# monkey0head/RePlay_cql

Hardware: AMD Instinct MI355X
Metric: CQL train-steps/sec (higher is better)
Workload: dtype bf16; 1 GPU; BASELINE.json configs[2]: synthetic 1000000 users x 100000 items, CQL d=128, L=50, B=4096/GPU, bf16 MFMA + fp32 accumulate; users=1000000, items=100000, d=128, window=50, batch_per_gpu=4096, global_batch=4096, parallelism=dp1 (users sharded by rank, RCCL gradient all-reduce), k=10, dp_variant=single

## Files before the change

### include/cqlrec.h

```cpp
#ifndef CQLREC_H
#define CQLREC_H
#include <stdint.h>
#ifdef __cplusplus
extern "C" {
#endif

#define CQLREC_OK 0
#define CQLREC_ERR_INVALID (-1)
#define CQLREC_ERR_HIP (-2)
#define CQLREC_ABI_VERSION 2
#define CQLREC_SEG_ALIGN 64

typedef void* cqlrec_stream;

int cqlrec_abi_version(void);
const char* cqlrec_last_error(void);

typedef struct cqlrec_layout {
  int64_t n_items;
  int32_t d;
  int32_t reserved;
  int64_t off_E_in, off_E_out, off_b_out, off_W1, off_b1, off_W2, off_b2;
  int64_t total;
} cqlrec_layout;
int cqlrec_layout_make(int64_t n_items, int32_t d, cqlrec_layout* out );

int cqlrec_sample_transitions(const int64_t* offsets, const int32_t* items, const float* rewards, int64_t n_users,
                              uint64_t seed, uint64_t step, uint64_t slot0, int32_t batch, int32_t* users,
                              int32_t* tpos, int32_t* act, float* rew, float* done, cqlrec_stream stream);

int cqlrec_gather_pool_fwd(const uint16_t* E_in_b, const int64_t* offsets, const int32_t* items,
                           const int32_t* users, const int32_t* ends, int32_t end_delta, int64_t n_states,
                           int32_t L, int32_t d, float* h0, uint16_t* h0_b, int32_t* lens, cqlrec_stream stream);
int cqlrec_gather_pool_bwd(const float* dh0, const int64_t* offsets, const int32_t* items, const int32_t* users,
                           const int32_t* ends, int32_t end_delta, int64_t n_states, int32_t L, int32_t d,
                           float* g_E_in, cqlrec_stream stream);
int64_t cqlrec_gather_pool_bwd_ws_bytes(int64_t n_states, int32_t L, int32_t d);
int cqlrec_gather_pool_bwd_prepare(const int64_t* offsets, const int32_t* items, const int32_t* users,
                                   const int32_t* ends, int32_t end_delta, int64_t n_states, int32_t L, int32_t d,
                                   int64_t n_items, void* ws, int64_t ws_bytes, cqlrec_stream stream);
int cqlrec_gather_pool_bwd_apply(const float* dh0, int64_t n_states, int32_t L, int32_t d, int64_t n_items, void* ws,
                                 int64_t ws_bytes, float* g_E_in, cqlrec_stream stream);
int cqlrec_gather_pool_bwd_sorted(const float* dh0, const int64_t* offsets, const int32_t* items,
                                  const int32_t* users, const int32_t* ends, int32_t end_delta, int64_t n_states,
                                  int32_t L, int32_t d, int64_t n_items, void* ws, int64_t ws_bytes,
                                  float* g_E_in, cqlrec_stream stream);

int cqlrec_linear_bf16(const uint16_t* X_b, const uint16_t* W_b, const float* bias, int64_t rows, int32_t d,
                       int32_t relu, float* Y, uint16_t* Y_b, cqlrec_stream stream);
int cqlrec_encoder_fwd(const uint16_t* X_b, const uint16_t* W1_b, const float* b1, const uint16_t* W2_b, const float* b2,
                       int64_t rows, int32_t d, uint16_t* Z_b, uint16_t* H_b, cqlrec_stream stream);
int64_t cqlrec_encoder_bwd_ws_bytes(int64_t rows, int32_t d);
int cqlrec_encoder_bwd(const float* dH, const uint16_t* z_b, const uint16_t* h0_b, const uint16_t* W1_b,
                       const uint16_t* W2_b, int64_t rows, int32_t d, void* ws, int64_t ws_bytes, float* g_W1,
                       float* g_b1, float* g_W2, float* g_b2, float* dh0, cqlrec_stream stream);

#define CQLREC_QHEAD_LSE 1
#define CQLREC_QHEAD_ARGMAX 2
int64_t cqlrec_qhead_ws_bytes(int64_t rows, int64_t n_items, int32_t d);
int cqlrec_qhead_fwd(const uint16_t* H_b, int64_t rows, const uint16_t* E_out_b, const float* b_out,
                     int64_t n_items, int32_t d, int32_t mode, void* ws, int64_t ws_bytes, float* out_val,
                     int32_t* out_idx, float* out_nlse2, cqlrec_stream stream);

int cqlrec_gather_dot(const uint16_t* H_b, const uint16_t* E_b, const float* b, const int32_t* idx, int64_t rows,
                      int32_t d, float* out, cqlrec_stream stream);

int cqlrec_td_loss(const float* q_a, const float* lse, const float* q_targ, const float* rew, const float* done,
                   int32_t batch, float gamma, float alpha, float inv_batch, float* coef, float* y,
                   float* loss_out, cqlrec_stream stream);
int64_t cqlrec_qhead_bwd_ws_bytes(int64_t batch, int64_t n_items, int32_t d);
int cqlrec_qhead_bwd(const uint16_t* H_b, const float* nlse2, const float* coef, const int32_t* act,
                     int64_t batch, const uint16_t* E_out_b, const float* b_out, int64_t n_items, int32_t d,
                     float scale, void* ws, int64_t ws_bytes, float* dH, float* g_E_out, float* g_b_out,
                     cqlrec_stream stream);

int cqlrec_qhead_bwd_items(const uint16_t* H_b, const float* nlse2, const float* coef, const int32_t* act,
                           int64_t batch, const uint16_t* E_out_b, const float* b_out, int64_t n_items, int32_t d,
                           float scale, void* ws, int64_t ws_bytes, float* g_E_out, float* g_b_out,
                           cqlrec_stream stream);
int cqlrec_qhead_bwd_states(const uint16_t* H_b, const float* nlse2, const float* coef, const int32_t* act,
                            int64_t batch, const uint16_t* E_out_b, const float* b_out, int64_t n_items, int32_t d,
                            float scale, void* ws, int64_t ws_bytes, float* dH, cqlrec_stream stream);

int64_t cqlrec_qhead_fused_ws_bytes(int64_t rows, int64_t n_items, int32_t d);
int cqlrec_qhead_fwd_lse_dh(const uint16_t* H_b, int64_t rows, const uint16_t* E_out_b, const float* b_out,
                            int64_t n_items, int32_t d, void* ws, int64_t ws_bytes, float* out_lse,
                            float* out_nlse2 , cqlrec_stream stream);
int cqlrec_qhead_dh_finish(const void* ws, int64_t rows, int64_t n_items, int32_t d, const float* lse,
                           const float* coef, const int32_t* act, const uint16_t* E_out_b, float scale, float* dH,
                           cqlrec_stream stream);

int cqlrec_adam_ema(float* theta, float* grads, float* m, float* v, float* target, uint16_t* theta_b,
                    uint16_t* target_b, int64_t n, float step_size, float sqrt_bc2, float beta1, float beta2,
                    float eps, float tau, int32_t zero_grads, cqlrec_stream stream);
int cqlrec_cast_bf16(const float* src, uint16_t* dst_b, int64_t n, cqlrec_stream stream);

int64_t cqlrec_topk_ws_bytes(int64_t n_users, int64_t n_cand, int32_t d, int32_t k);
int cqlrec_score_topk(const uint16_t* H_b, int64_t n_users, const uint16_t* E_b, const float* b, int64_t n_cand,
                      int32_t d, const int32_t* item_ids, const int64_t* seen_off, const int32_t* seen_items,
                      const int32_t* seen_rows, int32_t k, void* ws, int64_t ws_bytes, int32_t* out_idx,
                      float* out_val, int32_t* out_cnt, cqlrec_stream stream);
#define CQLREC_TOPK_ALL 0
#define CQLREC_TOPK_SEEN 1
#define CQLREC_TOPK_SCORE 2
// ... 339 lines not shown
```

### replay_cql_amd/_native.py

```python
from __future__ import annotations

import ctypes as C
import os
from pathlib import Path
from typing import Optional

os.environ.setdefault("GPU_MAX_HW_QUEUES", "8")

_LIB_PATH = Path(os.environ["CQLREC_LIB"]).resolve() if os.environ.get("CQLREC_LIB") else \
    Path(__file__).resolve().parent / "libcqlrec.so"
_lib: Optional[C.CDLL] = None

ABI_VERSION = 2
TOPK_ALL, TOPK_SEEN, TOPK_SCORE, TOPK_SEEN_BESIDE = 0, 1, 2, 3
SIM_DOT, SIM_COSINE, SIM_EUCLID = 0, 1, 2
ITEM_KNN_MAX_K = 512
PAIRS_MAX_K = 512
QHEAD_LSE = 1
QHEAD_ARGMAX = 2
EVAL_EXTRAS = ("RocAuc", "Unexpectedness", "Surprisal", "NCISPrecision")
NCIS_NONE, NCIS_SIGMOID, NCIS_SOFTMAX = 0, 1, 2

vp, i32, i64, u64, f32, f64 = C.c_void_p, C.c_int32, C.c_int64, C.c_uint64, C.c_float, C.c_double


class Layout(C.Structure):
    _fields_ = [
        ("n_items", i64), ("d", i32), ("reserved", i32),
        ("off_E_in", i64), ("off_E_out", i64), ("off_b_out", i64), ("off_W1", i64), ("off_b1", i64),
        ("off_W2", i64), ("off_b2", i64), ("total", i64),
    ]

    SEGMENTS = ("E_in", "E_out", "b_out", "W1", "b1", "W2", "b2")

    def offset(self, name: str) -> int:
        return int(getattr(self, "off_" + name))

    def shape(self, name: str):
        n, d = int(self.n_items), int(self.d)
        return {"E_in": (n + 1, d), "E_out": (n, d), "b_out": (n,), "W1": (d, d), "b1": (d,), "W2": (d, d),
                "b2": (d,)}[name]


class TrainCtx(C.Structure):
    _fields_ = [
        ("layout", Layout),
        ("offsets", vp), ("items", vp), ("rewards", vp), ("n_users", i64),
        ("theta", vp), ("grads", vp), ("adam_m", vp), ("adam_v", vp), ("target", vp), ("theta_b", vp),
        ("target_b", vp),
        ("batch", i32), ("window", i32), ("world", i32), ("rank", i32),
        ("gamma", f64), ("alpha", f64), ("lr", f64), ("beta1", f64), ("beta2", f64), ("eps", f64), ("tau", f64),
        ("seed", u64),
        ("ws", vp), ("ws_bytes", i64),
    ]


class TrainViews(C.Structure):
    _fields_ = [(n, vp) for n in (
        "users", "tpos", "act", "a_star", "rew", "done", "q_a", "lse", "q_targ", "y", "coef", "dH", "dh0", "h0_s",
        "hb_s", "hb_sn", "hb_tn")]


class FeaturesPop(C.Structure):
    _fields_ = [("code", vp), ("pair_code", vp), ("keys", vp), ("pop", vp), ("entity_off", vp), ("n_code", i64), ("n_entity", i64),
                ("n_cat", i64), ("m", i64), ("entity_is_item", i32), ("reserved", i32)]


FEATURES_STATS, FEATURES_MAX_COLS, FEATURES_MAX_POP = 6, 64, 8
FEAT_MEAN_GATHER, FEAT_MEAN_ABNORMALITY, FEAT_MEAN_ABNORMALITY_CR = 0, 1, 2
(FEAT_COL_USER, FEAT_COL_ITEM, FEAT_COL_NA_USER, FEAT_COL_NA_ITEM, FEAT_COL_DIFF_USER, FEAT_COL_DIFF_ITEM, FEAT_COL_POP,
 FEAT_COL_POP_NA) = range(8)

NEIGHBOUR_FIT, NEIGHBOUR_PREDICT = 0, 1
NEIGHBOUR_MAX_K = 1024
NEIGHBOUR_WEIGHTINGS = {None: 0, "tf_idf": 1, "bm25": 2}

ALS_PIECE, ALS_GRAM_BLOCK, ALS_MAX_RANK, ALS_MAX_K = 1024, 4096, 128, 512
ALS_EXPLICIT, ALS_IMPLICIT = 0, 1

SIGNATURES = {
    "cqlrec_abi_version": (i32, []),
    "cqlrec_last_error": (C.c_char_p, []),
    "cqlrec_layout_make": (i32, [i64, i32, C.POINTER(Layout)]),
    "cqlrec_sample_transitions": (i32, [vp, vp, vp, i64, u64, u64, u64, i32, vp, vp, vp, vp, vp, vp]),
    "cqlrec_gather_pool_fwd": (i32, [vp, vp, vp, vp, vp, i32, i64, i32, i32, vp, vp, vp, vp]),
    "cqlrec_gather_pool_bwd": (i32, [vp, vp, vp, vp, vp, i32, i64, i32, i32, vp, vp]),
    "cqlrec_gather_pool_bwd_ws_bytes": (i64, [i64, i32, i32]),
    "cqlrec_gather_pool_bwd_prepare": (i32, [vp, vp, vp, vp, i32, i64, i32, i32, i64, vp, i64, vp]),
    "cqlrec_gather_pool_bwd_apply": (i32, [vp, i64, i32, i32, i64, vp, i64, vp, vp]),
    "cqlrec_gather_pool_bwd_sorted": (i32, [vp, vp, vp, vp, vp, i32, i64, i32, i32, i64, vp, i64, vp, vp]),
    "cqlrec_linear_bf16": (i32, [vp, vp, vp, i64, i32, i32, vp, vp, vp]),
    "cqlrec_encoder_fwd": (i32, [vp, vp, vp, vp, vp, i64, i32, vp, vp, vp]),
    "cqlrec_encoder_bwd_ws_bytes": (i64, [i64, i32]),
    "cqlrec_encoder_bwd": (i32, [vp, vp, vp, vp, vp, i64, i32, vp, i64, vp, vp, vp, vp, vp, vp]),
    "cqlrec_qhead_ws_bytes": (i64, [i64, i64, i32]),
    "cqlrec_qhead_fwd": (i32, [vp, i64, vp, vp, i64, i32, i32, vp, i64, vp, vp, vp, vp]),
    "cqlrec_gather_dot": (i32, [vp, vp, vp, vp, i64, i32, vp, vp]),
    "cqlrec_td_loss": (i32, [vp, vp, vp, vp, vp, i32, f32, f32, f32, vp, vp, vp, vp]),
    "cqlrec_qhead_bwd_ws_bytes": (i64, [i64, i64, i32]),
    "cqlrec_qhead_bwd": (i32, [vp, vp, vp, vp, i64, vp, vp, i64, i32, f32, vp, i64, vp, vp, vp, vp]),
    "cqlrec_qhead_bwd_items": (i32, [vp, vp, vp, vp, i64, vp, vp, i64, i32, f32, vp, i64, vp, vp, vp]),
    "cqlrec_qhead_bwd_states": (i32, [vp, vp, vp, vp, i64, vp, vp, i64, i32, f32, vp, i64, vp, vp]),
    "cqlrec_adam_ema": (i32, [vp, vp, vp, vp, vp, vp, vp, i64, f32, f32, f32, f32, f32, f32, i32, vp]),
    "cqlrec_cast_bf16": (i32, [vp, vp, i64, vp]),
    "cqlrec_topk_ws_bytes": (i64, [i64, i64, i32, i32]),
    "cqlrec_score_topk": (i32, [vp, i64, vp, vp, i64, i32, vp, vp, vp, vp, i32, vp, i64, vp, vp, vp, vp]),
    "cqlrec_topk_seen_form": (i32, [vp, i64, i64, i32, i32, C.POINTER(C.c_int32), vp]),
    "cqlrec_score_topk_phase": (i32, [vp, i64, vp, vp, i64, i32, vp, vp, vp, vp, i32, vp, i64, vp, vp, vp, i32, vp]),
    "cqlrec_item_norms": (i32, [vp, i64, i32, vp, vp]),
    "cqlrec_item_knn_ws_bytes": (i64, [i64, i64, i32, i32]),
    "cqlrec_item_knn": (i32, [vp, vp, i64, i32, vp, i64, vp, i64, i32, i32, vp, i64, vp, vp, vp, vp]),
    "cqlrec_pairs_topk_ws_bytes": (i64, [i64, i64, i32, i32]),
    "cqlrec_pairs_topk": (i32, [vp, vp, vp, i64, i32, vp, vp, vp, i64, vp, vp, i32, vp, i64, vp, vp, vp, vp, vp]),
    "cqlrec_train_ws_bytes": (i64, [i32, i64, i32, i32]),
    "cqlrec_train_step_fwd_bwd": (i32, [C.POINTER(TrainCtx), u64, vp, vp]),
    "cqlrec_train_step_update": (i32, [C.POINTER(TrainCtx), u64, vp]),
    "cqlrec_train_step_forward": (i32, [C.POINTER(TrainCtx), u64, vp, vp]),
    "cqlrec_train_step_forward_after": (i32, [C.POINTER(TrainCtx), u64, vp, vp, vp]),
    "cqlrec_train_step_forward_early_items": (i32, [C.POINTER(TrainCtx), u64, vp, vp, vp, vp]),
    "cqlrec_train_step_backward_items": (i32, [C.POINTER(TrainCtx), u64, vp]),
    "cqlrec_train_step_backward_rest": (i32, [C.POINTER(TrainCtx), u64, vp]),
    "cqlrec_train_step_update_range": (i32, [C.POINTER(TrainCtx), u64, i64, i64, vp]),
    "cqlrec_set_concurrency": (i32, [i32]),
    "cqlrec_runtime_init": (i32, []),
    "cqlrec_runtime_probe_count": (i32, []),
    "cqlrec_aux_stream": (vp, [i32]),
    "cqlrec_qhead_fused_ws_bytes": (i64, [i64, i64, i32]),
    "cqlrec_qhead_fwd_lse_dh": (i32, [vp, i64, vp, vp, i64, i32, vp, i64, vp, vp, vp]),
    "cqlrec_qhead_dh_finish": (i32, [vp, i64, i64, i32, vp, vp, vp, vp, C.c_float, vp, vp]),
    "cqlrec_train_steps": (i32, [C.POINTER(TrainCtx), u64, i32, vp, vp]),
    "cqlrec_train_views_get": (i32, [C.POINTER(TrainCtx), u64, C.POINTER(TrainViews)]),
    "cqlrec_build_csr_ws_bytes": (i64, [i64]),
    "cqlrec_build_csr": (i32, [vp, vp, vp, vp, i64, i64, vp, i64, vp, vp, vp, vp]),
    "cqlrec_eval_topk_ws_bytes": (i64, [i64, i32]),
    "cqlrec_eval_topk": (i32, [vp, i64, i32, vp, vp, vp, C.POINTER(i32), i32, vp, i64, vp, vp, vp]),
    "cqlrec_recs_frame_to_block_ws_bytes": (i64, [i64, i64]),
    "cqlrec_recs_frame_to_block": (i32, [vp, vp, vp, vp, i64, i64, i32, i32, vp, i64, vp, vp, vp, vp, vp]),
    "cqlrec_recs_join_prev": (i32, [vp, vp, i64, vp, vp, i64, vp, vp]),
# ... 143 lines not shown
```

### replay_cql_amd/csrc/common.h

```cpp
#pragma once
#include <hip/hip_runtime.h>
#include <stdint.h>
#include <stdio.h>
#include <stdarg.h>

#include "../../include/cqlrec.h"

typedef __attribute__((ext_vector_type(8))) __bf16 bf16x8;
typedef __attribute__((ext_vector_type(4))) __bf16 bf16x4;
typedef __attribute__((ext_vector_type(16))) float f32x16;
typedef __attribute__((ext_vector_type(4))) float f32x4;
typedef __attribute__((address_space(3))) bf16x4 lds_bf16x4;

#define CQL_WAVE 64
#define CQL_LOG2E 1.4426950408889634f
#define CQL_LN2 0.6931471805599453f
#define NEG_INF_F (-__builtin_inff())

void cql_set_error(const char* fmt, ...);
#define CQL_REQUIRE(cond, ...)            \
  do {                                    \
    if (!(cond)) {                        \
      cql_set_error(__VA_ARGS__);         \
      return CQLREC_ERR_INVALID;          \
    }                                     \
  } while (0)
#define CQL_LAUNCH_CHECK(name)                                              \
  do {                                                                      \
    hipError_t e__ = hipGetLastError();                                     \
    if (e__ != hipSuccess) {                                                \
      cql_set_error("%s: launch failed: %s", name, hipGetErrorString(e__)); \
      return CQLREC_ERR_HIP;                                                \
    }                                                                       \
  } while (0)

#define CQL_MAX_DEVICES 16
static inline int cql_device_slot() {
  int dev = 0;
  if (hipGetDevice(&dev) != hipSuccess || dev < 0) dev = 0;
  return dev % CQL_MAX_DEVICES;
}

void cql_prof_begin(int phase, hipStream_t s);
void cql_prof_end(hipStream_t s);
struct CqlProfScope {
  hipStream_t s;
  CqlProfScope(int phase, hipStream_t st) : s(st) { cql_prof_begin(phase, st); }
  ~CqlProfScope() { cql_prof_end(s); }
};

int cql_encoder_bwd_parts(const float* dH, const uint16_t* z_b, const uint16_t* h0_b, const uint16_t* W1_b,
                          const uint16_t* W2_b, int64_t rows, int32_t d, void* ws, int64_t ws_bytes, float* g_W1, float* g_b1,
                          float* g_W2, float* g_b2, float* dh0, int parts, hipStream_t s);
int cql_td_coef(const float* q_a, const float* lse, const float* q_targ, const float* rew, const float* done, int32_t batch,
                float gamma, float alpha, float inv_batch, float* coef, float* y, float* term, hipStream_t s);
int cql_td_loss_sum(const float* term, int32_t batch, float inv_batch, float* loss_out, hipStream_t s);
int64_t cql_onehot_ws_bytes(int64_t batch, int32_t d);
int cql_onehot_prepare(const int32_t* act, int64_t batch, int64_t n_items, int32_t d, void* ws, int64_t ws_bytes,
                       hipStream_t s);
int cql_onehot_apply(const float* coef, const uint16_t* H_b, int64_t batch, int64_t n_items, int32_t d, void* ws,
                     float* g_E_out, float* g_b_out, hipStream_t s, int accumulate = 0);

static inline int cql_ceil_div(int64_t a, int64_t b) { return (int)((a + b - 1) / b); }
static inline int64_t cql_align256(int64_t x) { return (x + 255) / 256 * 256; }

__device__ __forceinline__ float bf16_bits_to_f32(uint16_t b) { return __uint_as_float(((uint32_t)b) << 16); }
__device__ __forceinline__ uint16_t f32_to_bf16_bits(float f) {
  __bf16 b = (__bf16)f;
  return __builtin_bit_cast(uint16_t, b);
}
__device__ __forceinline__ float bf16_round_f32(float f) { return bf16_bits_to_f32(f32_to_bf16_bits(f)); }

__device__ __forceinline__ void unpack_bf16x8(const uint4& v, float (&o)[8]) {
  o[0] = __uint_as_float(v.x << 16);
  o[1] = __uint_as_float(v.x & 0xFFFF0000u);
  o[2] = __uint_as_float(v.y << 16);
  o[3] = __uint_as_float(v.y & 0xFFFF0000u);
  o[4] = __uint_as_float(v.z << 16);
  o[5] = __uint_as_float(v.z & 0xFFFF0000u);
  o[6] = __uint_as_float(v.w << 16);
  o[7] = __uint_as_float(v.w & 0xFFFF0000u);
}
__device__ __forceinline__ uint32_t pack_bf16x2(float lo, float hi) {
  return (uint32_t)f32_to_bf16_bits(lo) | ((uint32_t)f32_to_bf16_bits(hi) << 16);
}

__device__ __forceinline__ int mfma_row(int reg, int half) { return (reg & 3) + 8 * (reg >> 2) + 4 * half; }

template <int D>
__device__ __forceinline__ int swz_chunk(int row, int ch) {
  if constexpr (D == 64) return ch ^ ((row >> 1) & 7);
  else return ch ^ (row & 15);
}

__device__ __forceinline__ float fast_exp2(float x) { return __builtin_amdgcn_exp2f(x); }

__device__ __forceinline__ uint32_t f32_order_key(float f) {
  uint32_t u = __float_as_uint(f);
  return (u & 0x80000000u) ? ~u : (u | 0x80000000u);
}
// ... 30 lines not shown
```

### replay_cql_amd/csrc/misc.hip

```cpp
#include <stdlib.h>
#include "common.h"
#include "adam_math.h"

static thread_local char g_err[512] = "";
void cql_set_error(const char* fmt, ...) {
  va_list ap;
  va_start(ap, fmt);
  vsnprintf(g_err, sizeof(g_err), fmt, ap);
  va_end(ap);
}
extern "C" const char* cqlrec_last_error(void) { return g_err; }
extern "C" int cqlrec_abi_version(void) { return CQLREC_ABI_VERSION; }

#define CQL_PROF_POOL 8192
static struct {
  bool on = false;
  bool created = false;
  hipEvent_t ev[CQL_PROF_POOL][2];
  int phase[CQL_PROF_POOL];
  int n = 0;
  int open = -1;
  uint32_t mask = 0xFFFFFFFFu;
} g_prof;

void cql_prof_begin(int phase, hipStream_t s) {
  if (!g_prof.on || g_prof.n >= CQL_PROF_POOL || !((g_prof.mask >> phase) & 1u)) return;
  g_prof.open = g_prof.n++;
  g_prof.phase[g_prof.open] = phase;
  (void)hipEventRecord(g_prof.ev[g_prof.open][0], s);
}
void cql_prof_end(hipStream_t s) {
  if (!g_prof.on || g_prof.open < 0) return;
  (void)hipEventRecord(g_prof.ev[g_prof.open][1], s);
  g_prof.open = -1;
}
extern "C" int cqlrec_prof_select(uint32_t phase_mask) {
  g_prof.mask = phase_mask;
  return CQLREC_OK;
}
extern "C" int cqlrec_prof_enable(int32_t on) {
  if (on && !g_prof.created) {
    for (int i = 0; i < CQL_PROF_POOL; ++i)
      for (int k = 0; k < 2; ++k)
        if (hipEventCreate(&g_prof.ev[i][k]) != hipSuccess) {
          cql_set_error("prof_enable: hipEventCreate failed");
          return CQLREC_ERR_HIP;
        }
    g_prof.created = true;
  }
  g_prof.on = on != 0;
  g_prof.n = 0;
  g_prof.open = -1;
  return CQLREC_OK;
}
extern "C" int cqlrec_prof_read(double* ms_sum, int64_t* launches) {
  CQL_REQUIRE(ms_sum && launches, "prof_read: NULL pointer");
  for (int p = 0; p < CQLREC_PH_COUNT; ++p) {
    ms_sum[p] = 0.0;
    launches[p] = 0;
  }
  for (int i = 0; i < g_prof.n; ++i) {
    float ms = 0.f;
    if (hipEventSynchronize(g_prof.ev[i][1]) != hipSuccess ||
        hipEventElapsedTime(&ms, g_prof.ev[i][0], g_prof.ev[i][1]) != hipSuccess) {
      cql_set_error("prof_read: event query failed");
      return CQLREC_ERR_HIP;
    }
    ms_sum[g_prof.phase[i]] += ms;
    launches[g_prof.phase[i]] += 1;
  }
  g_prof.n = 0;
  return CQLREC_OK;
}

extern "C" int cqlrec_layout_make(int64_t n_items, int32_t d, cqlrec_layout* out) {
  CQL_REQUIRE(out != nullptr, "layout_make: out is NULL");
  CQL_REQUIRE(n_items > 0 && n_items < (1ll << 31) - 64, "layout_make: n_items=%lld out of range", (long long)n_items);
  CQL_REQUIRE(d == 64 || d == 128 || d == 256, "layout_make: d=%d unsupported (64, 128 or 256)", d);
  int64_t sizes[7] = {(n_items + 1) * d, n_items * d, n_items, (int64_t)d * d, d, (int64_t)d * d, d};
  int64_t offs[7], cur = 0;
  for (int i = 0; i < 7; ++i) {
    offs[i] = cur;
    cur += (sizes[i] + CQLREC_SEG_ALIGN - 1) / CQLREC_SEG_ALIGN * CQLREC_SEG_ALIGN;
  }
  out->n_items = n_items;
  out->d = d;
  out->reserved = 0;
  out->off_E_in = offs[0];
  out->off_E_out = offs[1];
  out->off_b_out = offs[2];
  out->off_W1 = offs[3];
  out->off_b1 = offs[4];
  out->off_W2 = offs[5];
  out->off_b2 = offs[6];
  out->total = cur;
  return CQLREC_OK;
}

__host__ __device__ static inline uint64_t mix64(uint64_t z) {
  z += 0x9E3779B97F4A7C15ull;
  z = (z ^ (z >> 30)) * 0xBF58476D1CE4E5B9ull;
  z = (z ^ (z >> 27)) * 0x94D049BB133111EBull;
  return z ^ (z >> 31);
}

__global__ void sample_kernel(const int64_t* __restrict__ offsets, const int32_t* __restrict__ items,
                              const float* __restrict__ rewards, int64_t n_users, uint64_t k1, uint64_t slot0,
                              int batch, int32_t* users, int32_t* tpos, int32_t* act, float* rew, float* done) {
  int b = blockIdx.x * blockDim.x + threadIdx.x;
  if (b >= batch) return;
  const uint64_t nnz = (uint64_t)offsets[n_users];
  const uint64_t k2 = mix64(k1 + slot0 + (uint64_t)b);
  const int64_t p = (int64_t)__umul64hi(k2, nnz);
  int64_t lo = 0, hi = n_users;
  while (hi - lo > 1) {
    int64_t mid = (lo + hi) >> 1;
    if (offsets[mid] <= p) lo = mid; else hi = mid;
  }
  const int64_t o0 = offsets[lo], o1 = offsets[lo + 1];
  users[b] = (int32_t)lo;
  tpos[b] = (int32_t)(p - o0);
  act[b] = items[p];
  rew[b] = rewards[p];
  done[b] = (p == o1 - 1) ? 1.0f : 0.0f;
}

extern "C" int cqlrec_sample_transitions(const int64_t* offsets, const int32_t* items, const float* rewards,
                                         int64_t n_users, uint64_t seed, uint64_t step, uint64_t slot0,
                                         int32_t batch, int32_t* users, int32_t* tpos, int32_t* act, float* rew,
                                         float* done, cqlrec_stream stream) {
  CQL_REQUIRE(offsets && items && rewards && users && tpos && act && rew && done, "sample_transitions: NULL pointer");
  CQL_REQUIRE(n_users > 0 && batch > 0, "sample_transitions: n_users=%lld batch=%d", (long long)n_users, batch);
  const uint64_t k1 = mix64(seed ^ (step * 0xD1B54A32D192ED03ull));
  CqlProfScope prof(CQLREC_PH_SAMPLE, (hipStream_t)stream);
  hipLaunchKernelGGL(sample_kernel, dim3(cql_ceil_div(batch, 256)), dim3(256), 0, (hipStream_t)stream, offsets, items,
                     rewards, n_users, k1, slot0, batch, users, tpos, act, rew, done);
  CQL_LAUNCH_CHECK("sample_transitions");
  return CQLREC_OK;
}

template <int D>
__global__ __launch_bounds__(256) void gather_pool_fwd_kernel(const uint16_t* __restrict__ E_in_b,
                                                              const int64_t* __restrict__ offsets,
                                                              const int32_t* __restrict__ items,
                                                              const int32_t* __restrict__ users,
                                                              const int32_t* __restrict__ ends, int end_delta,
                                                              int64_t n_states, int L, float* __restrict__ h0,
                                                              uint16_t* __restrict__ h0_b, int32_t* __restrict__ lens) {
  constexpr int LPR = D / 8;
  constexpr int RPI = 64 / LPR;
  const int lane = threadIdx.x & 63;
  const int64_t state = (int64_t)blockIdx.x * 4 + (threadIdx.x >> 6);
  if (state >= n_states) return;
  const int u = users[state];
  const int64_t o0 = offsets[u];
  const int end = ends ? (ends[state] + end_delta) : (int)(offsets[u + 1] - o0);
  const int len = end < L ? end : L;
  const int32_t* win = items + o0 + end - len;
  const int slot = lane / LPR, c = lane % LPR;

  float acc[8];
#pragma unroll
  for (int i = 0; i < 8; ++i) acc[i] = 0.f;

  for (int j0 = 0; j0 < len; j0 += 4 * RPI) {
    int it[4];
    uint4 v[4];
#pragma unroll
    for (int q = 0; q < 4; ++q) {
      const int j = j0 + q * RPI + slot;
      it[q] = (j < len) ? win[j] : -1;
    }
#pragma unroll
    for (int q = 0; q < 4; ++q) {
      if (it[q] >= 0) v[q] = *reinterpret_cast<const uint4*>(E_in_b + (int64_t)it[q] * D + c * 8);
      else v[q] = make_uint4(0, 0, 0, 0);
    }
#pragma unroll
    for (int q = 0; q < 4; ++q) {
      float f[8];
      unpack_bf16x8(v[q], f);
#pragma unroll
      for (int i = 0; i < 8; ++i) acc[i] += f[i];
    }
  }
#pragma unroll
  for (int off = LPR; off < 64; off <<= 1) {
#pragma unroll
    for (int i = 0; i < 8; ++i) acc[i] += __shfl_xor(acc[i], off);
  }
  if (slot == 0) {
    const float fl = (float)len;
#pragma unroll
    for (int i = 0; i < 8; ++i) acc[i] = (len > 0) ? acc[i] / fl : 0.f;
    if (h0) {
      float4* o = reinterpret_cast<float4*>(h0 + state * D + c * 8);
      o[0] = make_float4(acc[0], acc[1], acc[2], acc[3]);
      o[1] = make_float4(acc[4], acc[5], acc[6], acc[7]);
    }
    if (h0_b) {
      uint4 p;
      p.x = pack_bf16x2(acc[0], acc[1]);
      p.y = pack_bf16x2(acc[2], acc[3]);
      p.z = pack_bf16x2(acc[4], acc[5]);
      p.w = pack_bf16x2(acc[6], acc[7]);
      *reinterpret_cast<uint4*>(h0_b + state * D + c * 8) = p;
    }
    if (lens && c == 0) lens[state] = len;
  }
}

extern "C" int cqlrec_gather_pool_fwd(const uint16_t* E_in_b, const int64_t* offsets, const int32_t* items,
                                      const int32_t* users, const int32_t* ends, int32_t end_delta, int64_t n_states,
                                      int32_t L, int32_t d, float* h0, uint16_t* h0_b, int32_t* lens,
                                      cqlrec_stream stream) {
  CQL_REQUIRE(E_in_b && offsets && items && users, "gather_pool_fwd: NULL pointer");
  CQL_REQUIRE(n_states >= 0 && L > 0, "gather_pool_fwd: n_states=%lld L=%d", (long long)n_states, L);
  CQL_REQUIRE(d == 64 || d == 128 || d == 256, "gather_pool_fwd: d=%d unsupported", d);
  if (n_states == 0) return CQLREC_OK;
  dim3 grid(cql_ceil_div(n_states, 4)), block(256);
  hipStream_t s = (hipStream_t)stream;
  CqlProfScope prof(CQLREC_PH_GATHER_FWD, s);
#define GP_LAUNCH(DD)                                                                                          \
  hipLaunchKernelGGL(gather_pool_fwd_kernel<DD>, grid, block, 0, s, E_in_b, offsets, items, users, ends, end_delta, \
                     n_states, L, h0, h0_b, lens)
  if (d == 64) GP_LAUNCH(64); else if (d == 128) GP_LAUNCH(128); else GP_LAUNCH(256);
#undef GP_LAUNCH
  CQL_LAUNCH_CHECK("gather_pool_fwd");
  return CQLREC_OK;
}

template <int D>
__global__ __launch_bounds__(256) void gather_pool_bwd_kernel(const float* __restrict__ dh0,
                                                              const int64_t* __restrict__ offsets,
                                                              const int32_t* __restrict__ items,
                                                              const int32_t* __restrict__ users,
                                                              const int32_t* __restrict__ ends, int end_delta,
                                                              int64_t n_states, int L, float* __restrict__ g_E_in) {
  constexpr int PER = D / 64;
  const int lane = threadIdx.x & 63;
  const int64_t state = (int64_t)blockIdx.x * 4 + (threadIdx.x >> 6);
  if (state >= n_states) return;
  const int u = users[state];
  const int64_t o0 = offsets[u];
  const int end = ends ? (ends[state] + end_delta) : (int)(offsets[u + 1] - o0);
  const int len = end < L ? end : L;
  if (len == 0) return;
  const int32_t* win = items + o0 + end - len;
  float g[PER];
  const float fl = (float)len;
#pragma unroll
  for (int k = 0; k < PER; ++k) g[k] = dh0[state * D + k * 64 + lane] / fl;
  for (int j = 0; j < len; ++j) {
    float* row = g_E_in + (int64_t)win[j] * D;
#pragma unroll
    for (int k = 0; k < PER; ++k) atomicAdd(row + k * 64 + lane, g[k]);
  }
}

extern "C" int cqlrec_gather_pool_bwd(const float* dh0, const int64_t* offsets, const int32_t* items,
                                      const int32_t* users, const int32_t* ends, int32_t end_delta, int64_t n_states,
                                      int32_t L, int32_t d, float* g_E_in, cqlrec_stream stream) {
  CQL_REQUIRE(dh0 && offsets && items && users && g_E_in, "gather_pool_bwd: NULL pointer");
  CQL_REQUIRE(d == 64 || d == 128 || d == 256, "gather_pool_bwd: d=%d unsupported", d);
  if (n_states <= 0) return CQLREC_OK;
  dim3 grid(cql_ceil_div(n_states, 4)), block(256);
  hipStream_t s = (hipStream_t)stream;
  CqlProfScope prof(CQLREC_PH_GATHER_BWD, s);
#define GB_LAUNCH(DD)                                                                                              \
  hipLaunchKernelGGL(gather_pool_bwd_kernel<DD>, grid, block, 0, s, dh0, offsets, items, users, ends, end_delta, \
                     n_states, L, g_E_in)
  if (d == 64) GB_LAUNCH(64); else if (d == 128) GB_LAUNCH(128); else GB_LAUNCH(256);
#undef GB_LAUNCH
  CQL_LAUNCH_CHECK("gather_pool_bwd");
  return CQLREC_OK;
}

template <int D>
__global__ __launch_bounds__(64) void linear_bf16_kernel(const uint16_t* __restrict__ X, const uint16_t* __restrict__ W,
                                                         const float* __restrict__ bias, int64_t rows, int relu,
                                                         float* __restrict__ Y, uint16_t* __restrict__ Yb) {
  constexpr int KS = D / 16;
  const int lane = threadIdx.x, r = lane & 31, h = lane >> 5;
  const int64_t m0 = (int64_t)blockIdx.x * 32;
  int64_t mrow = m0 + r;
  if (mrow >= rows) mrow = rows - 1;
  bf16x8 xf[KS];
#pragma unroll
  for (int s = 0; s < KS; ++s) xf[s] = *reinterpret_cast<const bf16x8*>(X + mrow * D + 16 * s + 8 * h);
#pragma unroll 1
  for (int ot = 0; ot < D / 32; ++ot) {
    const int o = ot * 32 + r;
    const float bo = bias[o];
    f32x16 acc;
#pragma unroll
    for (int i = 0; i < 16; ++i) acc[i] = bo;
#pragma unroll
    for (int s = 0; s < KS; ++s) {
      bf16x8 wf = *reinterpret_cast<const bf16x8*>(W + (int64_t)o * D + 16 * s + 8 * h);
      acc = __builtin_amdgcn_mfma_f32_32x32x16_bf16(xf[s], wf, acc, 0, 0, 0);
    }
#pragma unroll
    for (int i = 0; i < 16; ++i) {
      const int64_t m = m0 + mfma_row(i, h);
      float v = acc[i];
      if (relu) v = fmaxf(v, 0.f);
      if (m < rows) {
        if (Y) Y[m * D + o] = v;
        if (Yb) Yb[m * D + o] = f32_to_bf16_bits(v);
      }
    }
  }
}

template <int D>
__global__ __launch_bounds__(64) void encoder_fwd_kernel(const uint16_t* __restrict__ X, const uint16_t* __restrict__ W1,
                                                         const float* __restrict__ b1, const uint16_t* __restrict__ W2,
                                                         const float* __restrict__ b2, int64_t rows,
                                                         uint16_t* __restrict__ Zb, uint16_t* __restrict__ Hb) {
  constexpr int KS = D / 16;
  constexpr int LDZ = D + 8;
  __shared__ __attribute__((aligned(16))) uint16_t zt[32 * LDZ];
  const int lane = threadIdx.x, r = lane & 31, h = lane >> 5;
  const int64_t m0 = (int64_t)blockIdx.x * 32;
  int64_t mrow = m0 + r;
  if (mrow >= rows) mrow = rows - 1;
  bf16x8 xf[KS];
#pragma unroll
  for (int s = 0; s < KS; ++s) xf[s] = *reinterpret_cast<const bf16x8*>(X + mrow * D + 16 * s + 8 * h);
#pragma unroll 1
  for (int ot = 0; ot < D / 32; ++ot) {
    const int o = ot * 32 + r;
    const float bo = b1[o];
    f32x16 acc;
#pragma unroll
    for (int i = 0; i < 16; ++i) acc[i] = bo;
#pragma unroll
    for (int s = 0; s < KS; ++s) {
      bf16x8 wf = *reinterpret_cast<const bf16x8*>(W1 + (int64_t)o * D + 16 * s + 8 * h);
      acc = __builtin_amdgcn_mfma_f32_32x32x16_bf16(xf[s], wf, acc, 0, 0, 0);
    }
#pragma unroll
    for (int i = 0; i < 16; ++i) {
      const int mr = mfma_row(i, h);
      const uint16_t zb = f32_to_bf16_bits(fmaxf(acc[i], 0.f));
      zt[mr * LDZ + o] = zb;
      if (m0 + mr < rows) Zb[(m0 + mr) * D + o] = zb;
    }
  }
  __syncthreads();
  bf16x8 zf[KS];
#pragma unroll
  for (int s = 0; s < KS; ++s) zf[s] = *reinterpret_cast<const bf16x8*>(zt + r * LDZ + 16 * s + 8 * h);
#pragma unroll 1
  for (int ot = 0; ot < D / 32; ++ot) {
    const int o = ot * 32 + r;
    const float bo = b2[o];
    f32x16 acc;
#pragma unroll
    for (int i = 0; i < 16; ++i) acc[i] = bo;
#pragma unroll
    for (int s = 0; s < KS; ++s) {
      bf16x8 wf = *reinterpret_cast<const bf16x8*>(W2 + (int64_t)o * D + 16 * s + 8 * h);
      acc = __builtin_amdgcn_mfma_f32_32x32x16_bf16(zf[s], wf, acc, 0, 0, 0);
    }
#pragma unroll
    for (int i = 0; i < 16; ++i) {
      const int64_t m = m0 + mfma_row(i, h);
      if (m < rows) Hb[m * D + o] = f32_to_bf16_bits(acc[i]);
    }
  }
}

extern "C" int cqlrec_encoder_fwd(const uint16_t* X_b, const uint16_t* W1_b, const float* b1, const uint16_t* W2_b,
                                  const float* b2, int64_t rows, int32_t d, uint16_t* Z_b, uint16_t* H_b,
                                  cqlrec_stream stream) {
  CQL_REQUIRE(X_b && W1_b && b1 && W2_b && b2 && Z_b && H_b, "encoder_fwd: NULL pointer");
  CQL_REQUIRE(d == 64 || d == 128 || d == 256, "encoder_fwd: d=%d unsupported", d);
  if (rows <= 0) return CQLREC_OK;
  dim3 grid(cql_ceil_div(rows, 32)), block(64);
  hipStream_t s = (hipStream_t)stream;
  CqlProfScope prof(CQLREC_PH_ENCODER_FWD, s);
#define ENCF_LAUNCH(DD) hipLaunchKernelGGL(encoder_fwd_kernel<DD>, grid, block, 0, s, X_b, W1_b, b1, W2_b, b2, rows, Z_b, H_b)
  if (d == 64) ENCF_LAUNCH(64); else if (d == 128) ENCF_LAUNCH(128); else ENCF_LAUNCH(256);
#undef ENCF_LAUNCH
  CQL_LAUNCH_CHECK("encoder_fwd");
  return CQLREC_OK;
}

extern "C" int cqlrec_linear_bf16(const uint16_t* X_b, const uint16_t* W_b, const float* bias, int64_t rows, int32_t d,
                                  int32_t relu, float* Y, uint16_t* Y_b, cqlrec_stream stream) {
  CQL_REQUIRE(X_b && W_b && bias, "linear_bf16: NULL pointer");
  CQL_REQUIRE(d == 64 || d == 128 || d == 256, "linear_bf16: d=%d unsupported", d);
  if (rows <= 0) return CQLREC_OK;
  dim3 grid(cql_ceil_div(rows, 32)), block(64);
  hipStream_t s = (hipStream_t)stream;
  CqlProfScope prof(CQLREC_PH_ENCODER_FWD, s);
#define LIN_LAUNCH(DD) hipLaunchKernelGGL(linear_bf16_kernel<DD>, grid, block, 0, s, X_b, W_b, bias, rows, relu, Y, Y_b)
  if (d == 64) LIN_LAUNCH(64); else if (d == 128) LIN_LAUNCH(128); else LIN_LAUNCH(256);
#undef LIN_LAUNCH
  CQL_LAUNCH_CHECK("linear_bf16");
  return CQLREC_OK;
}

template <int D>
__global__ __launch_bounds__(256) void enc_bwd_dx_kernel(const float* __restrict__ dH, const uint16_t* __restrict__ zb,
                                                         const uint16_t* __restrict__ W1b,
                                                         const uint16_t* __restrict__ W2b, int64_t rows,
                                                         float* __restrict__ dA1, float* __restrict__ dh0) {
  constexpr int LD = D + 1;
  constexpr int NT = D / 32;
  __shared__ float tile[2][32 * LD];
  const int t = threadIdx.x, lane = t & 63, wave = t >> 6;
  const int r = lane & 31, h = lane >> 5;
  const int64_t m0 = (int64_t)blockIdx.x * 32;
  for (int i = t; i < 32 * D; i += 256) {
    const int rr = i / D, cc = i % D;
    tile[0][rr * LD + cc] = (m0 + rr < rows) ? dH[(m0 + rr) * D + cc] : 0.f;
  }
  __syncthreads();
  for (int nt = wave; nt < NT; nt += 4) {
    f32x16 acc;
#pragma unroll
    for (int i = 0; i < 16; ++i) acc[i] = 0.f;
#pragma unroll 8
    for (int s = 0; s < D / 2; ++s) {
      const int o = 2 * s + h;
      const float a = tile[0][r * LD + o];
      const float bv = bf16_bits_to_f32(W2b[(int64_t)o * D + nt * 32 + r]);
      acc = __builtin_amdgcn_mfma_f32_32x32x2f32(a, bv, acc, 0, 0, 0);
    }
#pragma unroll
    for (int i = 0; i < 16; ++i) {
      const int rr = mfma_row(i, h), col = nt * 32 + r;
      const int64_t m = m0 + rr;
      float v = 0.f;
      if (m < rows) {
// ... 474 lines not shown
```

Before: 1552 train-steps/s (B=4096 transitions per step and GPU).

## Batch gather-pool and encoder forward into multi-job launches; multi-wave encoder

Adds job-table variants of the gather-pool and encoder forward kernels that process up to four independent jobs in one launch via blockIdx.y. The encoder forward for d=64/128 becomes a multi-wave kernel where each wave owns output tiles, preloads its weights into registers and stores through LDS with coalesced vector writes, and Z output becomes optional. The goal is fewer launches and better per-block parallelism. It changes nothing unless callers use the multi entry points, and the single-job encoder path now always runs the new kernel.

```diff
diff --git a/include/cqlrec.h b/include/cqlrec.h
--- a/include/cqlrec.h
+++ b/include/cqlrec.h
@@ -32,6 +32,19 @@
 int cqlrec_gather_pool_fwd(const uint16_t* E_in_b, const int64_t* offsets, const int32_t* items,
                            const int32_t* users, const int32_t* ends, int32_t end_delta, int64_t n_states,
                            int32_t L, int32_t d, float* h0, uint16_t* h0_b, int32_t* lens, cqlrec_stream stream);
+#define CQLREC_MAX_JOBS 4
+typedef struct cqlrec_gather_job {
+  const uint16_t* E_in_b;
+  const int32_t* ends;
+  float* h0;
+  uint16_t* h0_b;
+  int32_t* lens;
+  int32_t end_delta;
+  int32_t reserved;
+} cqlrec_gather_job;
+int cqlrec_gather_pool_fwd_multi(const cqlrec_gather_job* jobs , int32_t n_jobs,
+                                 const int64_t* offsets, const int32_t* items, const int32_t* users, int64_t n_states,
+                                 int32_t L, int32_t d, cqlrec_stream stream);
 int cqlrec_gather_pool_bwd(const float* dh0, const int64_t* offsets, const int32_t* items, const int32_t* users,
                            const int32_t* ends, int32_t end_delta, int64_t n_states, int32_t L, int32_t d,
                            float* g_E_in, cqlrec_stream stream);
@@ -50,6 +63,17 @@
                        int32_t relu, float* Y, uint16_t* Y_b, cqlrec_stream stream);
 int cqlrec_encoder_fwd(const uint16_t* X_b, const uint16_t* W1_b, const float* b1, const uint16_t* W2_b, const float* b2,
                        int64_t rows, int32_t d, uint16_t* Z_b, uint16_t* H_b, cqlrec_stream stream);
+typedef struct cqlrec_encoder_job {
+  const uint16_t* X_b;
+  const uint16_t* W1_b;
+  const float* b1;
+  const uint16_t* W2_b;
+  const float* b2;
+  uint16_t* Z_b;
+  uint16_t* H_b;
+} cqlrec_encoder_job;
+int cqlrec_encoder_fwd_multi(const cqlrec_encoder_job* jobs , int32_t n_jobs, int64_t rows, int32_t d,
+                             cqlrec_stream stream);
 int64_t cqlrec_encoder_bwd_ws_bytes(int64_t rows, int32_t d);
 int cqlrec_encoder_bwd(const float* dH, const uint16_t* z_b, const uint16_t* h0_b, const uint16_t* W1_b,
                        const uint16_t* W2_b, int64_t rows, int32_t d, void* ws, int64_t ws_bytes, float* g_W1,
diff --git a/replay_cql_amd/_native.py b/replay_cql_amd/_native.py
--- a/replay_cql_amd/_native.py
+++ b/replay_cql_amd/_native.py
@@ -61,6 +61,17 @@
         "hb_s", "hb_sn", "hb_tn")]
 
 
+MAX_JOBS = 4
+
+
+class GatherJob(C.Structure):
+    _fields_ = [("E_in_b", vp), ("ends", vp), ("h0", vp), ("h0_b", vp), ("lens", vp), ("end_delta", i32), ("reserved", i32)]
+
+
+class EncoderJob(C.Structure):
+    _fields_ = [("X_b", vp), ("W1_b", vp), ("b1", vp), ("W2_b", vp), ("b2", vp), ("Z_b", vp), ("H_b", vp)]
+
+
 class FeaturesPop(C.Structure):
     _fields_ = [("code", vp), ("pair_code", vp), ("keys", vp), ("pop", vp), ("entity_off", vp), ("n_code", i64), ("n_entity", i64),
                 ("n_cat", i64), ("m", i64), ("entity_is_item", i32), ("reserved", i32)]
@@ -84,6 +95,8 @@
     "cqlrec_layout_make": (i32, [i64, i32, C.POINTER(Layout)]),
     "cqlrec_sample_transitions": (i32, [vp, vp, vp, i64, u64, u64, u64, i32, vp, vp, vp, vp, vp, vp]),
     "cqlrec_gather_pool_fwd": (i32, [vp, vp, vp, vp, vp, i32, i64, i32, i32, vp, vp, vp, vp]),
+    "cqlrec_gather_pool_fwd_multi": (i32, [C.POINTER(GatherJob), i32, vp, vp, vp, i64, i32, i32, vp]),
+    "cqlrec_encoder_fwd_multi": (i32, [C.POINTER(EncoderJob), i32, i64, i32, vp]),
     "cqlrec_gather_pool_bwd": (i32, [vp, vp, vp, vp, vp, i32, i64, i32, i32, vp, vp]),
     "cqlrec_gather_pool_bwd_ws_bytes": (i64, [i64, i32, i32]),
     "cqlrec_gather_pool_bwd_prepare": (i32, [vp, vp, vp, vp, i32, i64, i32, i32, i64, vp, i64, vp]),
diff --git a/replay_cql_amd/csrc/common.h b/replay_cql_amd/csrc/common.h
--- a/replay_cql_amd/csrc/common.h
+++ b/replay_cql_amd/csrc/common.h
@@ -41,11 +41,11 @@
   return dev % CQL_MAX_DEVICES;
 }
 
-void cql_prof_begin(int phase, hipStream_t s);
+void cql_prof_begin(int phase, hipStream_t s, int launches = 1);
 void cql_prof_end(hipStream_t s);
 struct CqlProfScope {
   hipStream_t s;
-  CqlProfScope(int phase, hipStream_t st) : s(st) { cql_prof_begin(phase, st); }
+  CqlProfScope(int phase, hipStream_t st, int launches = 1) : s(st) { cql_prof_begin(phase, st, launches); }
   ~CqlProfScope() { cql_prof_end(s); }
 };
 
diff --git a/replay_cql_amd/csrc/misc.hip b/replay_cql_amd/csrc/misc.hip
--- a/replay_cql_amd/csrc/misc.hip
+++ b/replay_cql_amd/csrc/misc.hip
@@ -18,15 +18,17 @@
   bool created = false;
   hipEvent_t ev[CQL_PROF_POOL][2];
   int phase[CQL_PROF_POOL];
+  int launches[CQL_PROF_POOL];
   int n = 0;
   int open = -1;
   uint32_t mask = 0xFFFFFFFFu;
 } g_prof;
 
-void cql_prof_begin(int phase, hipStream_t s) {
+void cql_prof_begin(int phase, hipStream_t s, int launches) {
   if (!g_prof.on || g_prof.n >= CQL_PROF_POOL || !((g_prof.mask >> phase) & 1u)) return;
   g_prof.open = g_prof.n++;
   g_prof.phase[g_prof.open] = phase;
+  g_prof.launches[g_prof.open] = launches;
   (void)hipEventRecord(g_prof.ev[g_prof.open][0], s);
 }
 void cql_prof_end(hipStream_t s) {
@@ -67,7 +69,7 @@
       return CQLREC_ERR_HIP;
     }
     ms_sum[g_prof.phase[i]] += ms;
-    launches[g_prof.phase[i]] += 1;
+    launches[g_prof.phase[i]] += g_prof.launches[i];
   }
   g_prof.n = 0;
   return CQLREC_OK;
@@ -139,19 +141,26 @@
   return CQLREC_OK;
 }
 
-template <int D>
-__global__ __launch_bounds__(256) void gather_pool_fwd_kernel(const uint16_t* __restrict__ E_in_b,
+struct CqlGatherJobs { cqlrec_gather_job j[CQLREC_MAX_JOBS]; };
+struct CqlEncoderJobs { cqlrec_encoder_job j[CQLREC_MAX_JOBS]; };
+
+template <int D>
+__global__ __launch_bounds__(256) void gather_pool_fwd_kernel(const CqlGatherJobs jobs,
                                                               const int64_t* __restrict__ offsets,
                                                               const int32_t* __restrict__ items,
-                                                              const int32_t* __restrict__ users,
-                                                              const int32_t* __restrict__ ends, int end_delta,
-                                                              int64_t n_states, int L, float* __restrict__ h0,
-                                                              uint16_t* __restrict__ h0_b, int32_t* __restrict__ lens) {
+                                                              const int32_t* __restrict__ users, int64_t n_states, int L) {
   constexpr int LPR = D / 8;
   constexpr int RPI = 64 / LPR;
   const int lane = threadIdx.x & 63;
   const int64_t state = (int64_t)blockIdx.x * 4 + (threadIdx.x >> 6);
   if (state >= n_states) return;
+  const cqlrec_gather_job& job = jobs.j[blockIdx.y];
+  const uint16_t* __restrict__ E_in_b = job.E_in_b;
+  const int32_t* __restrict__ ends = job.ends;
+  const int end_delta = job.end_delta;
+  float* __restrict__ h0 = job.h0;
+  uint16_t* __restrict__ h0_b = job.h0_b;
+  int32_t* __restrict__ lens = job.lens;
   const int u = users[state];
   const int64_t o0 = offsets[u];
   const int end = ends ? (ends[state] + end_delta) : (int)(offsets[u + 1] - o0);
@@ -214,16 +223,28 @@
                                       const int32_t* users, const int32_t* ends, int32_t end_delta, int64_t n_states,
                                       int32_t L, int32_t d, float* h0, uint16_t* h0_b, int32_t* lens,
                                       cqlrec_stream stream) {
-  CQL_REQUIRE(E_in_b && offsets && items && users, "gather_pool_fwd: NULL pointer");
+  const cqlrec_gather_job job = {E_in_b, ends, h0, h0_b, lens, end_delta, 0};
+  return cqlrec_gather_pool_fwd_multi(&job, 1, offsets, items, users, n_states, L, d, stream);
+}
+
+extern "C" int cqlrec_gather_pool_fwd_multi(const cqlrec_gather_job* jobs, int32_t n_jobs, const int64_t* offsets,
+                                            const int32_t* items, const int32_t* users, int64_t n_states, int32_t L,
+                                            int32_t d, cqlrec_stream stream) {
+  CQL_REQUIRE(jobs && n_jobs >= 1 && n_jobs <= CQLREC_MAX_JOBS, "gather_pool_fwd: n_jobs=%d (1..%d)", n_jobs,
+              CQLREC_MAX_JOBS);
+  CQL_REQUIRE(offsets && items && users, "gather_pool_fwd: NULL pointer");
+  CqlGatherJobs tab = {};
+  for (int j = 0; j < n_jobs; ++j) {
+    CQL_REQUIRE(jobs[j].E_in_b != nullptr, "gather_pool_fwd: NULL pointer");
+    tab.j[j] = jobs[j];
+  }
   CQL_REQUIRE(n_states >= 0 && L > 0, "gather_pool_fwd: n_states=%lld L=%d", (long long)n_states, L);
   CQL_REQUIRE(d == 64 || d == 128 || d == 256, "gather_pool_fwd: d=%d unsupported", d);
   if (n_states == 0) return CQLREC_OK;
-  dim3 grid(cql_ceil_div(n_states, 4)), block(256);
+  dim3 grid(cql_ceil_div(n_states, 4), n_jobs), block(256);
   hipStream_t s = (hipStream_t)stream;
-  CqlProfScope prof(CQLREC_PH_GATHER_FWD, s);
-#define GP_LAUNCH(DD)                                                                                          \
-  hipLaunchKernelGGL(gather_pool_fwd_kernel<DD>, grid, block, 0, s, E_in_b, offsets, items, users, ends, end_delta, \
-                     n_states, L, h0, h0_b, lens)
+  CqlProfScope prof(CQLREC_PH_GATHER_FWD, s, n_jobs);
+#define GP_LAUNCH(DD) hipLaunchKernelGGL(gather_pool_fwd_kernel<DD>, grid, block, 0, s, tab, offsets, items, users, n_states, L)
   if (d == 64) GP_LAUNCH(64); else if (d == 128) GP_LAUNCH(128); else GP_LAUNCH(256);
 #undef GP_LAUNCH
   CQL_LAUNCH_CHECK("gather_pool_fwd");
@@ -314,13 +335,103 @@
 }
 
 template <int D>
-__global__ __launch_bounds__(64) void encoder_fwd_kernel(const uint16_t* __restrict__ X, const uint16_t* __restrict__ W1,
-                                                         const float* __restrict__ b1, const uint16_t* __restrict__ W2,
-                                                         const float* __restrict__ b2, int64_t rows,
-                                                         uint16_t* __restrict__ Zb, uint16_t* __restrict__ Hb) {
+struct EncGeom {
+  static constexpr int KS = D / 16, LDZ = D + 8, NT = D / 32, NW = NT < 4 ? NT : 4, TPW = NT / NW, NTH = NW * 64;
+};
+
+template <int D>
+__device__ __forceinline__ void enc_store_tile(const uint16_t* zt, uint16_t* __restrict__ G, int64_t m0, int64_t rows) {
+  constexpr int CPR = D / 8;
+  for (int idx = threadIdx.x; idx < 32 * CPR; idx += EncGeom<D>::NTH) {
+    const int row = idx / CPR, ch = idx % CPR;
+    if (m0 + row < rows)
+      *reinterpret_cast<uint4*>(G + (m0 + row) * D + ch * 8) =
+          *reinterpret_cast<const uint4*>(zt + row * EncGeom<D>::LDZ + ch * 8);
+  }
+}
+
+template <int D>
+__device__ __forceinline__ void enc_load_w(bf16x8 (&wf)[D / 16], float& bo, const uint16_t* __restrict__ W,
+                                           const float* __restrict__ bias, int o, int h) {
+#pragma unroll
+  for (int s = 0; s < D / 16; ++s) wf[s] = *reinterpret_cast<const bf16x8*>(W + (int64_t)o * D + 16 * s + 8 * h);
+  bo = bias[o];
+}
+template <int D>
+__device__ __forceinline__ f32x16 enc_chain(const bf16x8 (&af)[D / 16], const bf16x8 (&wf)[D / 16], float bo) {
+  f32x16 acc;
+#pragma unroll
+  for (int i = 0; i < 16; ++i) acc[i] = bo;
+#pragma unroll
+  for (int s = 0; s < D / 16; ++s) acc = __builtin_amdgcn_mfma_f32_32x32x16_bf16(af[s], wf[s], acc, 0, 0, 0);
+  return acc;
+}
+
+template <int D>
+__global__ __launch_bounds__(EncGeom<D>::NTH) void encoder_fwd_kernel(const CqlEncoderJobs jobs, int64_t rows) {
+  using G = EncGeom<D>;
+  constexpr int KS = G::KS, LDZ = G::LDZ, TPW = G::TPW;
+  __shared__ __attribute__((aligned(16))) uint16_t zt[32 * LDZ];
+  const cqlrec_encoder_job& job = jobs.j[blockIdx.y];
+  const uint16_t* __restrict__ X = job.X_b;
+  uint16_t* __restrict__ Zb = job.Z_b;
+  const int lane = threadIdx.x & 63, r = lane & 31, h = lane >> 5;
+  const int wv = __builtin_amdgcn_readfirstlane(threadIdx.x >> 6);
+  const int64_t m0 = (int64_t)blockIdx.x * 32;
+  int64_t mrow = m0 + r;
+  if (mrow >= rows) mrow = rows - 1;
+  bf16x8 xf[KS], w1f[TPW][KS], w2f[TPW][KS];
+  float bo1[TPW], bo2[TPW];
+#pragma unroll
+  for (int s = 0; s < KS; ++s) xf[s] = *reinterpret_cast<const bf16x8*>(X + mrow * D + 16 * s + 8 * h);
+#pragma unroll
+  for (int t = 0; t < TPW; ++t) enc_load_w<D>(w1f[t], bo1[t], job.W1_b, job.b1, (wv * TPW + t) * 32 + r, h);
+#pragma unroll
+  for (int t = 0; t < TPW; ++t) enc_load_w<D>(w2f[t], bo2[t], job.W2_b, job.b2, (wv * TPW + t) * 32 + r, h);
+  __builtin_amdgcn_sched_barrier(0);
+#pragma unroll
+  for (int t = 0; t < TPW; ++t) {
+    const int o = (wv * TPW + t) * 32 + r;
+    const f32x16 acc = enc_chain<D>(xf, w1f[t], bo1[t]);
+#pragma unroll
+    for (int i = 0; i < 16; ++i) zt[mfma_row(i, h) * LDZ + o] = f32_to_bf16_bits(fmaxf(acc[i], 0.f));
+  }
+  __syncthreads();
+  bf16x8 zf[KS];
+#pragma unroll
+  for (int s = 0; s < KS; ++s) zf[s] = *reinterpret_cast<const bf16x8*>(zt + r * LDZ + 16 * s + 8 * h);
+  if (Zb) enc_store_tile<D>(zt, Zb, m0, rows);
+  uint16_t hq[TPW][16];
+#pragma unroll
+  for (int t = 0; t < TPW; ++t) {
+    const f32x16 acc = enc_chain<D>(zf, w2f[t], bo2[t]);
+#pragma unroll
+    for (int i = 0; i < 16; ++i) hq[t][i] = f32_to_bf16_bits(acc[i]);
+  }
+  __syncthreads();
+#pragma unroll
+  for (int t = 0; t < TPW; ++t) {
+    const int o = (wv * TPW + t) * 32 + r;
+#pragma unroll
+    for (int i = 0; i < 16; ++i) zt[mfma_row(i, h) * LDZ + o] = hq[t][i];
+  }
+  __syncthreads();
+  enc_store_tile<D>(zt, job.H_b, m0, rows);
+}
+
+template <int D>
+__global__ __launch_bounds__(64) void encoder_fwd_1wave_kernel(const CqlEncoderJobs jobs, int64_t rows) {
   constexpr int KS = D / 16;
   constexpr int LDZ = D + 8;
   __shared__ __attribute__((aligned(16))) uint16_t zt[32 * LDZ];
+  const cqlrec_encoder_job& job = jobs.j[blockIdx.y];
+  const uint16_t* __restrict__ X = job.X_b;
+  const uint16_t* __restrict__ W1 = job.W1_b;
+  const uint16_t* __restrict__ W2 = job.W2_b;
+  const float* __restrict__ b1 = job.b1;
+  const float* __restrict__ b2 = job.b2;
+  uint16_t* __restrict__ Zb = job.Z_b;
+  uint16_t* __restrict__ Hb = job.H_b;
   const int lane = threadIdx.x, r = lane & 31, h = lane >> 5;
   const int64_t m0 = (int64_t)blockIdx.x * 32;
   int64_t mrow = m0 + r;
@@ -345,7 +456,7 @@
       const int mr = mfma_row(i, h);
       const uint16_t zb = f32_to_bf16_bits(fmaxf(acc[i], 0.f));
       zt[mr * LDZ + o] = zb;
-      if (m0 + mr < rows) Zb[(m0 + mr) * D + o] = zb;
+      if (Zb && m0 + mr < rows) Zb[(m0 + mr) * D + o] = zb;
     }
   }
   __syncthreads();
@@ -376,13 +487,30 @@
                                   const float* b2, int64_t rows, int32_t d, uint16_t* Z_b, uint16_t* H_b,
                                   cqlrec_stream stream) {
   CQL_REQUIRE(X_b && W1_b && b1 && W2_b && b2 && Z_b && H_b, "encoder_fwd: NULL pointer");
+  const cqlrec_encoder_job job = {X_b, W1_b, b1, W2_b, b2, Z_b, H_b};
+  return cqlrec_encoder_fwd_multi(&job, 1, rows, d, stream);
+}
+
+extern "C" int cqlrec_encoder_fwd_multi(const cqlrec_encoder_job* jobs, int32_t n_jobs, int64_t rows, int32_t d,
+                                        cqlrec_stream stream) {
+  CQL_REQUIRE(jobs && n_jobs >= 1 && n_jobs <= CQLREC_MAX_JOBS, "encoder_fwd: n_jobs=%d (1..%d)", n_jobs, CQLREC_MAX_JOBS);
+  CqlEncoderJobs tab = {};
+  for (int j = 0; j < n_jobs; ++j) {
+    const cqlrec_encoder_job& e = jobs[j];
+    CQL_REQUIRE(e.X_b && e.W1_b && e.b1 && e.W2_b && e.b2 && e.H_b, "encoder_fwd: NULL pointer");
+    CQL_REQUIRE(((uintptr_t)e.X_b | (uintptr_t)e.W1_b | (uintptr_t)e.W2_b | (uintptr_t)e.Z_b | (uintptr_t)e.H_b) % 16 == 0,
+                "encoder_fwd: X_b, W1_b, W2_b, Z_b and H_b must be 16-byte aligned");
+    tab.j[j] = e;
+  }
   CQL_REQUIRE(d == 64 || d == 128 || d == 256, "encoder_fwd: d=%d unsupported", d);
   if (rows <= 0) return CQLREC_OK;
-  dim3 grid(cql_ceil_div(rows, 32)), block(64);
+  dim3 grid(cql_ceil_div(rows, 32), n_jobs);
   hipStream_t s = (hipStream_t)stream;
-  CqlProfScope prof(CQLREC_PH_ENCODER_FWD, s);
-#define ENCF_LAUNCH(DD) hipLaunchKernelGGL(encoder_fwd_kernel<DD>, grid, block, 0, s, X_b, W1_b, b1, W2_b, b2, rows, Z_b, H_b)
-  if (d == 64) ENCF_LAUNCH(64); else if (d == 128) ENCF_LAUNCH(128); else ENCF_LAUNCH(256);
+  CqlProfScope prof(CQLREC_PH_ENCODER_FWD, s, n_jobs);
+#define ENCF_LAUNCH(DD) hipLaunchKernelGGL(encoder_fwd_kernel<DD>, grid, dim3(EncGeom<DD>::NTH), 0, s, tab, rows)
+  if (d == 64) ENCF_LAUNCH(64);
+  else if (d == 128) ENCF_LAUNCH(128);
+  else hipLaunchKernelGGL(encoder_fwd_1wave_kernel<256>, grid, dim3(64), 0, s, tab, rows);
 #undef ENCF_LAUNCH
   CQL_LAUNCH_CHECK("encoder_fwd");
   return CQLREC_OK;
```

Measured after the change: 1563 train-steps/s (B=4096 transitions per step and GPU), median of 3. No clear change (+0.8%).
